# TopJohn/corda

Measured on AMD Instinct MI355X. Metric: signature verifications/sec (whole node, 1/2/4/8 GPU) + % integer-ALU peak, higher is better.
Workload: dtype u32

## Files before the change

### corda_amd/csrc/ed25519.hip

```cpp
#ifndef FE_QUAD
#define FE_QUAD 0
#endif
#ifndef FE_USE_ASM2
#define FE_USE_ASM2 1
#endif
#include <hip/hip_runtime.h>

#include <functional>
#include <stdint.h>
#include <stdlib.h>

#include "ed25519_ops.hpp"
#include "ed25519_ws.hpp"
#include "sha2_device.hpp"
#include "status.hpp"

namespace cordahip {

__global__ void __launch_bounds__(64) ed25519_btable_kernel(uint32_t* __restrict__ tab) {
  const int g = blockIdx.x * blockDim.x + threadIdx.x;
  if (g >= 2 * kBTableEntries) return;
  const int k = g % kBTableEntries;
  ge_p3 B, P;
  ge_base(B);
  if (g >= kBTableEntries)
    for (int t = 0; t < kBDigits * kBBits; t++) ge_dbl<true>(B, B);
  ge_cached bc;
  ge_to_cached(bc, B);
  ge_identity(P);
  for (int bit = kBBits - 1; bit >= 0; bit--) {
    ge_dbl<true>(P, P);
    if ((k >> bit) & 1) ge_add<true>(P, P, bc);
  }
  store_niels_entry(tab + g * kBEntryWords, P);
}

CDEV bool mp8_ge(const uint32_t a[8], const uint32_t b[8]) {
  uint32_t br = 0;
#pragma unroll
  for (int i = 0; i < 8; i++) br = (uint32_t)(((uint64_t)a[i] - b[i] - br) >> 63);
  return br == 0;
}
CDEV void mp8_add(uint32_t r[8], const uint32_t a[8], const uint32_t b[8]) {
  uint64_t c = 0;
#pragma unroll
  for (int i = 0; i < 8; i++) {
    c += (uint64_t)a[i] + b[i];
    r[i] = (uint32_t)c;
    c >>= 32;
  }
}
CDEV void mp8_neg(uint32_t a[8]) {
  uint64_t c = 1;
#pragma unroll
  for (int i = 0; i < 8; i++) {
    c += (uint64_t)(~a[i]);
    a[i] = (uint32_t)c;
    c >>= 32;
  }
}
CDEV void mp8_copy(uint32_t d[8], const uint32_t s[8]) {
#pragma unroll
  for (int i = 0; i < 8; i++) d[i] = s[i];
}
CDEV int mp8_absbits(const uint32_t a[8]) {
  uint32_t t[8];
  mp8_copy(t, a);
  if (a[7] >> 31) mp8_neg(t);
  return mp8_bitlen(t);
}

CDEV double mp8_f64(const uint32_t a[8]) {
  double d = (double)a[7];
#pragma unroll
  for (int i = 6; i >= 0; i--) d = fma(d, 4294967296.0, (double)a[i]);
  return d;
}
CDEV void mp8_submul(uint32_t a[8], const uint32_t b[8], uint32_t q) {
  uint64_t pc = 0;
  uint32_t br = 0;
#pragma unroll
  for (int i = 0; i < 8; i++) {
    const uint64_t p = (uint64_t)q * b[i] + pc;
    pc = p >> 32;
    const uint64_t d = (uint64_t)a[i] - (uint32_t)p - br;
    a[i] = (uint32_t)d;
    br = (uint32_t)(d >> 63);
  }
}
CDEV void mp8_shl_dyn(uint32_t o[8], const uint32_t b[8], int k) {
  const int ws = k >> 5, bs = k & 31;
#pragma unroll
  for (int i = 0; i < 8; i++) {
    const uint32_t lo = (i - ws >= 0) ? word_sel(b, i - ws) : 0u;
    const uint32_t lo2 = (i - ws - 1 >= 0) ? word_sel(b, i - ws - 1) : 0u;
    o[i] = bs ? ((lo << bs) | (lo2 >> (32 - bs))) : lo;
  }
}

CDEV void euclid_divstep(uint32_t rp[8], const uint32_t rc[8], uint32_t tp[8], const uint32_t tc[8]) {
  const double inv = 1.0 / mp8_f64(rc);
  while (mp8_ge(rp, rc)) {
    const double qd = mp8_f64(rp) * inv * (1.0 - 0x1p-40);
    if (qd < 4294967296.0) {
      uint32_t q = (uint32_t)qd;
      q = q ? q : 1u;
      mp8_submul(rp, rc, q);
      mp8_submul(tp, tc, q);
    } else {
      const int e = (int)((__double_as_longlong(qd) >> 52) & 0x7ff) - 1023;
      const int k = e - 31;
      const uint32_t q = (uint32_t)(qd * __longlong_as_double((long long)(1023 - k) << 52));
      uint32_t bs[8], ts[8];
      mp8_shl_dyn(bs, rc, k);
      mp8_shl_dyn(ts, tc, k);
      mp8_submul(rp, bs, q);
      mp8_submul(tp, ts, q);
    }
  }
}

CDEV double mp8_top(const uint32_t a[8], int s) {
  const int w = s >> 5, b = s & 31;
  const uint64_t lo = ((uint64_t)word_sel(a, w + 1) << 32) | word_sel(a, w);
  const uint64_t hi = word_sel(a, w + 2);
  return (double)((lo >> b) | (b ? hi << (64 - b) : 0ull));
}
CDEV void mp8_lincomb(uint32_t o[8], const uint32_t x[8], int a, const uint32_t y[8], int b) {
  const uint32_t ua = (uint32_t)(a < 0 ? -a : a), ub = (uint32_t)(b < 0 ? -b : b);
  uint64_t pc = 0, qc = 0;
  uint32_t br = 0;
#pragma unroll
  for (int i = 0; i < 8; i++) {
    const uint64_t p = (uint64_t)ua * x[i] + pc;
    pc = p >> 32;
    const uint64_t q = (uint64_t)ub * y[i] + qc;
    qc = q >> 32;
    const uint64_t d = (uint64_t)(uint32_t)p - (uint32_t)q - br;
    o[i] = (uint32_t)d;
    br = (uint32_t)(d >> 63);
  }
  if (b > 0 || (b == 0 && a < 0)) mp8_neg(o);
}

CDEV void half_scalars(uint32_t c0abs[8], bool& c0neg, uint32_t c1[8], const uint32_t h[8]) {
  const uint32_t kM[8] = {0xe7ae9f68u, 0xc09318d2u, 0x17bce6b2u, 0xa6f7cef5u, 0u, 0u, 0u, 0x80000000u};
  const uint32_t kS[8] = {0x754abea0u, 0x597d89b3u, 0xf9de6484u, 0xb504f333u, 0u, 0u, 0u, 0u};
  uint32_t rp[8], rc[8], tp[8], tc[8];
#pragma unroll
  for (int i = 0; i < 8; i++) {
    rp[i] = kM[i];
    rc[i] = h[i];
    tp[i] = 0;
    tc[i] = i == 0;
  }
  for (;;) {
    const int s = max(mp8_bitlen(rp) - 52, 0);
    double uh = mp8_top(rp, s), vh = mp8_top(rc, s);
    const double th = mp8_top(kS, s) + 1.0;
    double A = 1.0, B = 0.0, C = 0.0, D = 1.0;
    int n = 0;
    for (;;) {
      const double d1 = vh + C, d2 = vh + D;
      if (!(d1 > 0.0 && d2 > 0.0)) break;
      const double n1 = uh + A;
      double q = floor(n1 / d1);
      const double r1 = fma(-q, d1, n1);
      q = r1 < 0.0 ? q - 1.0 : (r1 >= d1 ? q + 1.0 : q);
      const double r2 = fma(-q, d2, uh + B);
      if (!(r2 >= 0.0 && r2 < d2)) break;
      const double nC = fma(-q, C, A), nD = fma(-q, D, B), nv = fma(-q, vh, uh);
      const double mc = fmax(fabs(nC), fabs(nD));
      if (nv - mc < th || mc >= 0x1p30) break;
      A = C;
      B = D;
      C = nC;
      D = nD;
      uh = vh;
      vh = nv;
      n++;
    }
    if (n == 0) break;
    const int a = (int)A, b = (int)B, c = (int)C, d = (int)D;
    uint32_t x[8], y[8];
    mp8_lincomb(x, rp, a, rc, b);
    mp8_lincomb(y, rp, c, rc, d);
    mp8_copy(rp, x);
    mp8_copy(rc, y);
    mp8_lincomb(x, tp, a, tc, b);
    mp8_lincomb(y, tp, c, tc, d);
    mp8_copy(tp, x);
    mp8_copy(tc, y);
  }
  while (mp8_ge(rc, kS)) {
    euclid_divstep(rp, rc, tp, tc);
#pragma unroll
    for (int i = 0; i < 8; i++) {
      const uint32_t a = rp[i], b = tp[i];
      rp[i] = rc[i];
      rc[i] = a;
      tp[i] = tc[i];
      tc[i] = b;
    }
  }
  uint32_t a0[8], a1[8];
  mp8_copy(a0, rc);
  mp8_copy(a1, tc);
  if (!(tc[0] & 1)) {
    uint32_t r3[8], t3[8];
    mp8_copy(r3, rp);
    mp8_copy(t3, tp);
    euclid_divstep(r3, rc, t3, tc);
    uint32_t p0[8], p1[8], m0[8], m1[8], nr3[8], nt3[8];
    mp8_add(p0, rc, r3);
    mp8_add(p1, tc, t3);
    mp8_copy(nr3, r3);
    mp8_neg(nr3);
    mp8_copy(nt3, t3);
    mp8_neg(nt3);
    mp8_add(m0, rc, nr3);
    mp8_add(m1, tc, nt3);
    int best = max(mp8_absbits(r3), mp8_absbits(t3));
    mp8_copy(a0, r3);
    mp8_copy(a1, t3);
    const int bp = max(mp8_absbits(p0), mp8_absbits(p1));
    if (bp < best) {
      best = bp;
      mp8_copy(a0, p0);
      mp8_copy(a1, p1);
    }
    const int bm = max(mp8_absbits(m0), mp8_absbits(m1));
    if (bm < best) {
      mp8_copy(a0, m0);
      mp8_copy(a1, m1);
    }
  }
  if (a1[7] >> 31) {
    mp8_neg(a0);
    mp8_neg(a1);
  }
  c0neg = (a0[7] >> 31) != 0;
  if (c0neg) mp8_neg(a0);
  mp8_copy(c0abs, a0);
  mp8_copy(c1, a1);
}

CDEV bool ge_strict_ok(const ge_p3& R, const uint32_t w[8]) {
  uint32_t all_ones = (w[7] & 0x7fffffffu) == 0x7fffffffu;
#pragma unroll
  for (int i = 1; i < 7; i++) all_ones &= (w[i] == 0xffffffffu);
  if (all_ones && w[0] >= 0xffffffedu) return false;
  return !((w[7] >> 31) && fe_iszero(R.X));
}

CDEV void store_point(uint32_t* __restrict__ o, const ge_p3& p) {
  uint4* o4 = reinterpret_cast<uint4*>(o);
  uint32_t w[32];
#pragma unroll
  for (int i = 0; i < 10; i++) {
    w[i] = p.X.v[i];
    w[10 + i] = p.Y.v[i];
    w[20 + i] = p.T.v[i];
  }
  w[30] = w[31] = 0;
#pragma unroll
  for (int q = 0; q < 8; q++) o4[q] = make_uint4(w[4 * q], w[4 * q + 1], w[4 * q + 2], w[4 * q + 3]);
}
CDEV void load_point(ge_p3& p, const uint32_t* __restrict__ o) {
  const uint4* o4 = reinterpret_cast<const uint4*>(o);
  uint32_t w[32];
#pragma unroll
  for (int q = 0; q < 8; q++) {
    const uint4 v = o4[q];
    w[4 * q] = v.x;
    w[4 * q + 1] = v.y;
    w[4 * q + 2] = v.z;
    w[4 * q + 3] = v.w;
  }
#pragma unroll
  for (int i = 0; i < 10; i++) {
    p.X.v[i] = w[i];
    p.Y.v[i] = w[10 + i];
    p.T.v[i] = w[20 + i];
  }
  fe_set(p.Z, 1);
}

static constexpr int kParkP = joint_index(2, 2), kParkQ = joint_index(2, -2);

CDEV uint32_t* joint_slot(uint32_t* rec, int idx) { return rec + kWhTab + idx * kWhEntryWords; }

CDEV void load_cached_niels(ge_niels& n, const uint32_t* __restrict__ p) {
  ge_cached c;
  load_cached(c, p);
  n.ypx = c.YpX;
  n.ymx = c.YmX;
  n.xy2d = c.T2d;
}

CDEV void joint_single_pass(uint32_t* __restrict__ rec, int pass) {
  ge_p3 B, D;
  load_point(B, joint_slot(rec, pass ? kParkQ : kParkP));
  ge_cached c;
  ge_to_cached(c, B);
  store_cached(joint_slot(rec, pass ? joint_index(0, 1) : joint_index(1, 0)), c);
  ge_dbl<true>(D, B);
  ge_to_cached(c, D);
  store_cached(joint_slot(rec, pass ? joint_index(0, 2) : joint_index(2, 0)), c);
}

CDEV void joint_sign_pass(uint32_t* __restrict__ rec, int s) {
  ge_p3 D, E;
  ge_niels nq, np;
  ge_cached c;
  load_point(D, joint_slot(rec, kParkP));
  load_cached_niels(nq, joint_slot(rec, joint_index(0, 1)));
  niels_cneg(nq, s < 0);
  ge_madd<true>(D, D, nq);
  ge_to_cached(c, D);
  store_cached(joint_slot(rec, joint_index(1, s)), c);
  ge_madd<true>(E, D, nq);
  ge_to_cached(c, E);
  store_cached(joint_slot(rec, joint_index(1, 2 * s)), c);
  load_cached_niels(np, joint_slot(rec, joint_index(1, 0)));
  ge_madd<true>(E, D, np);
  ge_to_cached(c, E);
  store_cached(joint_slot(rec, joint_index(2, s)), c);
  ge_dbl<true>(E, D);
  ge_to_cached(c, E);
  store_cached(joint_slot(rec, joint_index(2, 2 * s)), c);
}


#ifndef ED_PREP_WAVES
#define ED_PREP_WAVES 2
#endif
CDEV uint8_t prep_decode_phase(const uint8_t* __restrict__ keys, const uint8_t* __restrict__ sigs, uint64_t i,
                               uint32_t msg_len, const uint8_t* __restrict__ pre_status, uint32_t empty_is_error,
                               uint32_t* __restrict__ rec, uint32_t abyte[8], uint32_t Rw[8]) {
  uint8_t st = kStatusPending;
  load8(Rw, reinterpret_cast<const uint32_t*>(sigs + i * 64));
  {
    uint32_t wa[8];
    load8(wa, reinterpret_cast<const uint32_t*>(keys + i * 32));
    ge_p3 A, R;
    bool okA, okR;
    ge_frombytes_i2p_pair(A, okA, wa, R, okR, Rw);
    if (!okA) st = kStatusBadKey;
    else if (pre_status && pre_status[i] != kStatusOk) st = pre_status[i];
    else if (msg_len == 0 && empty_is_error) st = kStatusEmpty;
    fe_tobytes(abyte, A.Y);
    abyte[7] |= fe_isnegative(A.X) << 31;
    if (st == kStatusPending && !(okR && ge_strict_ok(R, Rw))) st = kStatusBadSig;
    if (st != kStatusPending) {
      ge_identity(A);
      ge_identity(R);
    }
    fe_neg(A.X, A.X);
    fe_neg(A.T, A.T);
    fe_neg(R.X, R.X);
    fe_neg(R.T, R.T);
    store_point(joint_slot(rec, kParkP), A);
    store_point(joint_slot(rec, kParkQ), R);
  }
  return st;
}

CDEV void prep_table_phase(uint32_t* __restrict__ rec) {
#pragma unroll 1
  for (int pass = 0; pass < 2; pass++) {
    joint_single_pass(rec, pass);
    PHASE_BARRIER();
  }
#pragma unroll 1
  for (int s = -1; s <= 1; s += 2) {
    joint_sign_pass(rec, s);
    PHASE_BARRIER();
  }
}

CDEV uint8_t prep_keys_phase(const uint8_t* __restrict__ keys, const uint8_t* __restrict__ sigs, uint64_t i,
                             uint32_t msg_len, const uint8_t* __restrict__ pre_status, uint32_t empty_is_error,
                             uint32_t* __restrict__ rec, uint32_t abyte[8], uint32_t Rw[8]) {
  const uint8_t st = prep_decode_phase(keys, sigs, i, msg_len, pre_status, empty_is_error, rec, abyte, Rw);
  PHASE_BARRIER();
  prep_table_phase(rec);
  return st;
}

CDEV void prep_msg_phase(const uint8_t* __restrict__ sigs, const uint8_t* __restrict__ msgs, uint32_t msg_len,
                         uint64_t i, uint8_t st, const uint32_t abyte[8], const uint32_t Rw[8],
                         uint32_t* __restrict__ rec) {
  uint32_t ka[8], kr[8], e[8];
  bool c0neg = false;
  if (st == kStatusPending) {
    uint32_t S[8], hd[16], h[8], se[8], zero[8];
    load8(S, reinterpret_cast<const uint32_t*>(sigs + i * 64 + 32));
    sha512_segments(hd, Rw, abyte, true, msgs + i * (uint64_t)msg_len, msg_len);
    sc_reduce512(h, hd);
    sc_effective_S(se, S, slide_drops_carry(S));
    half_scalars(ka, c0neg, kr, h);
#pragma unroll
    for (int q = 0; q < 8; q++) zero[q] = 0;
    sc_muladd(e, kr, se, zero);
  } else {
#pragma unroll
    for (int q = 0; q < 8; q++) ka[q] = kr[q] = e[q] = 0;
  }
  store8(rec + kWhKa, ka);
  store8(rec + kWhKr, kr);
  store8(rec + kWhE, e);
  reinterpret_cast<uint4*>(rec + kWhFlags)[0] = make_uint4(c0neg ? 1u : 0u, 0u, 0u, 0u);
}

__global__ void __launch_bounds__(256) __attribute__((amdgpu_waves_per_eu(ED_PREP_WAVES))) ed25519_prep_half_kernel(
    const uint8_t* __restrict__ keys, const uint8_t* __restrict__ sigs, const uint8_t* __restrict__ msgs,
    uint32_t msg_len, uint64_t base, uint64_t m, const uint8_t* __restrict__ pre_status,
    uint8_t* __restrict__ status, uint32_t* __restrict__ ws, uint32_t empty_is_error) {
  const uint64_t li = (uint64_t)blockIdx.x * blockDim.x + threadIdx.x;
  if (li >= m) return;
  const uint64_t i = base + li;
  uint32_t* rec = ws + li * kWhLaneWords;
  uint32_t abyte[8], Rw[8];
  const uint8_t st = prep_keys_phase(keys, sigs, i, msg_len, pre_status, empty_is_error, rec, abyte, Rw);
  prep_msg_phase(sigs, msgs, msg_len, i, st, abyte, Rw, rec);
  status[i] = st;
}

__global__ void __launch_bounds__(256) __attribute__((amdgpu_waves_per_eu(ED_PREP_WAVES))) ed25519_prep_keys_kernel(
    const uint8_t* __restrict__ keys, const uint8_t* __restrict__ sigs, uint32_t msg_len, uint64_t base, uint64_t m,
    const uint8_t* __restrict__ pre_status, uint8_t* __restrict__ status, uint32_t* __restrict__ ws,
    uint32_t empty_is_error) {
  const uint64_t li = (uint64_t)blockIdx.x * blockDim.x + threadIdx.x;
  if (li >= m) return;
  const uint64_t i = base + li;
  uint32_t* rec = ws + li * kWhLaneWords;
  uint32_t abyte[8], Rw[8];
  status[i] = prep_keys_phase(keys, sigs, i, msg_len, pre_status, empty_is_error, rec, abyte, Rw);
  store8(rec + kWhKa, abyte);
}

__global__ void __launch_bounds__(256) __attribute__((amdgpu_waves_per_eu(ED_PREP_WAVES))) ed25519_prep_msg_kernel(const uint8_t* __restrict__ sigs,
                                                               const uint8_t* __restrict__ msgs, uint32_t msg_len,
                                                               uint64_t base, uint64_t m,
                                                               const uint8_t* __restrict__ status,
                                                               uint32_t* __restrict__ ws) {
  const uint64_t li = (uint64_t)blockIdx.x * blockDim.x + threadIdx.x;
  if (li >= m) return;
  const uint64_t i = base + li;
  uint32_t* rec = ws + li * kWhLaneWords;
  uint32_t abyte[8], Rw[8];
  load8(abyte, rec + kWhKa);
  load8(Rw, reinterpret_cast<const uint32_t*>(sigs + i * 64));
  prep_msg_phase(sigs, msgs, msg_len, i, status[i], abyte, Rw, rec);
}

CDEV void fixed_base_mult(ge_p3& P, const uint32_t k[8], const uint32_t* __restrict__ btab) {
  ge_identity(P);
  for (int j = 31; j >= 0; j--) {
    if (j != 31) {
#pragma unroll
      for (int t = 0; t < 7; t++) ge_dbl<false>(P, P);
      ge_dbl<true>(P, P);
    }
    const int d = booth_digit<8>(k, j);
    ge_niels nb;
    load_niels(nb, btab, d < 0 ? -d : d);
    niels_cneg(nb, d < 0);
    ge_madd<true>(P, P, nb);
  }
}

__global__ void __launch_bounds__(256) ed25519_sign_kernel(const uint8_t* __restrict__ seeds,
                                                          const uint8_t* __restrict__ msgs, uint32_t msg_len,
                                                          uint64_t n, const uint32_t* __restrict__ btab,
                                                          uint8_t* __restrict__ pubs, uint8_t* __restrict__ sigs) {
  const uint64_t i = (uint64_t)blockIdx.x * blockDim.x + threadIdx.x;
  if (i >= n) return;
  uint32_t seed[8];
  {
    const uint4* s4 = reinterpret_cast<const uint4*>(seeds + i * 32);
    const uint4 a = s4[0], b = s4[1];
    seed[0] = a.x; seed[1] = a.y; seed[2] = a.z; seed[3] = a.w;
    seed[4] = b.x; seed[5] = b.y; seed[6] = b.z; seed[7] = b.w;
  }
  const uint8_t* msg = msgs + i * (uint64_t)msg_len;
  uint32_t hs[16], dummy[8];
#pragma unroll
  for (int q = 0; q < 8; q++) dummy[q] = 0;
  sha512_segments(hs, seed, dummy, false, msg, 0);
  uint32_t a[8], prefix[8];
#pragma unroll
  for (int q = 0; q < 8; q++) {
    a[q] = hs[q];
    prefix[q] = hs[8 + q];
  }
  a[0] &= ~7u;
  a[7] &= 0x3fffffffu;
  a[7] |= 0x40000000u;
  uint32_t a16[16], ar[8];
#pragma unroll
  for (int q = 0; q < 8; q++) {
    a16[q] = a[q];
    a16[8 + q] = 0;
  }
  sc_reduce512(ar, a16);
  ge_p3 A;
  fixed_base_mult(A, ar, btab);
  uint32_t pub[8];
  ge_tobytes(pub, A);
  uint32_t rh[16], r[8];
  sha512_segments(rh, prefix, dummy, false, msg, msg_len);
  sc_reduce512(r, rh);
  ge_p3 Rp;
  fixed_base_mult(Rp, r, btab);
  uint32_t R[8];
  ge_tobytes(R, Rp);
  uint32_t kh[16], k[8], S[8];
  sha512_segments(kh, R, pub, true, msg, msg_len);
  sc_reduce512(k, kh);
  sc_muladd(S, k, ar, r);
  uint4* p4 = reinterpret_cast<uint4*>(pubs + i * 32);
  p4[0] = make_uint4(pub[0], pub[1], pub[2], pub[3]);
  p4[1] = make_uint4(pub[4], pub[5], pub[6], pub[7]);
  uint4* s4 = reinterpret_cast<uint4*>(sigs + i * 64);
  s4[0] = make_uint4(R[0], R[1], R[2], R[3]);
  s4[1] = make_uint4(R[4], R[5], R[6], R[7]);
  s4[2] = make_uint4(S[0], S[1], S[2], S[3]);
  s4[3] = make_uint4(S[4], S[5], S[6], S[7]);
}

}

namespace cordahip {
hipError_t launch_ed25519_btable(uint32_t* tab, hipStream_t s) {
  hipLaunchKernelGGL(ed25519_btable_kernel, dim3((2 * kBTableEntries + 63) / 64), dim3(64), 0, s, tab);
  return hipGetLastError();
}
size_t ed25519_btable_bytes() { return 2 * (size_t)kBTableEntries * kBEntryWords * sizeof(uint32_t); }

size_t ed25519_ws_lane_bytes() { return kWhLaneWords * sizeof(uint32_t); }

hipError_t launch_ed25519_verify(const uint8_t* keys, const uint8_t* sigs, const uint8_t* msgs, uint32_t msg_len,
                                 uint64_t n, const uint32_t* btab, const uint8_t* pre_status, uint8_t* status,
                                 unsigned long long* verdict, uint32_t* ws, uint64_t ws_lanes, uint32_t flags,
                                 hipStream_t s, const std::function<hipError_t()>* before_msgs) {
  if (n == 0) return hipSuccess;
  if (!ws || ws_lanes < 64 || ws_lanes % 64) return hipErrorInvalidValue;
  bool msgs_ready = before_msgs == nullptr;
  for (uint64_t base = 0; base < n; base += ws_lanes) {
    const uint64_t m = n - base < ws_lanes ? n - base : ws_lanes;
    const uint32_t blocks = (uint32_t)((m + 255) / 256);
    hipError_t e = hipSuccess;
    if (msgs_ready) {
      hipLaunchKernelGGL(ed25519_prep_half_kernel, dim3(blocks), dim3(256), 0, s, keys, sigs, msgs, msg_len, base, m,
                         pre_status, status, ws, (flags & 1u) ? 0u : 1u);
      e = hipGetLastError();
    } else {
      hipLaunchKernelGGL(ed25519_prep_keys_kernel, dim3(blocks), dim3(256), 0, s, keys, sigs, msg_len, base, m,
                         pre_status, status, ws, (flags & 1u) ? 0u : 1u);
      e = hipGetLastError();
      e = e ? e : (*before_msgs)();
      msgs_ready = true;
      if (e == hipSuccess)
        hipLaunchKernelGGL(ed25519_prep_msg_kernel, dim3(blocks), dim3(256), 0, s, sigs, msgs, msg_len, base, m, status,
                           ws);
      e = e ? e : hipGetLastError();
    }
    if (e == hipSuccess) e = launch_ed25519_ladder(base, m, btab, ws, status, verdict, s);
    if (e != hipSuccess) return e;
  }
  return hipSuccess;
}

hipError_t launch_ed25519_sign(const uint8_t* seeds, const uint8_t* msgs, uint32_t msg_len, uint64_t n,
                               const uint32_t* btab, uint8_t* pubs, uint8_t* sigs, hipStream_t s) {
  if (n == 0) return hipSuccess;
  const uint64_t blocks = (n + 255) / 256;
  hipLaunchKernelGGL(ed25519_sign_kernel, dim3((uint32_t)blocks), dim3(256), 0, s, seeds, msgs, msg_len, n, btab,
                     pubs, sigs);
  return hipGetLastError();
}
}
```

### corda_amd/csrc/ed25519_ladder.hip

```cpp
#ifndef FE_USE_ASM2
#define FE_USE_ASM2 1
#endif
#include <hip/hip_runtime.h>
#include <stdint.h>

#include "ed25519_ws.hpp"
#include "status.hpp"

namespace cordahip {

__device__ __attribute__((aligned(64))) const uint32_t kIdentityCached[kWhEntryWords] = {1, 0, 0, 0, 0, 0, 0, 0, 0, 0,
                                                            1, 0, 0, 0, 0, 0, 0, 0, 0, 0,
                                                            1, 0, 0, 0, 0, 0, 0, 0, 0, 0,
                                                            0, 0, 0, 0, 0, 0, 0, 0, 0, 0};

#ifndef ED_LADDER_WAVES
#define ED_LADDER_WAVES 2
#endif
static_assert(512 / ED_LADDER_WAVES >= 168, "fe25519_asm.hpp's v160..v167 accumulators need >= 168 VGPRs per lane");

__global__ void __launch_bounds__(256) __attribute__((amdgpu_waves_per_eu(ED_LADDER_WAVES))) ed25519_ladder_half_kernel(
    uint64_t base, uint64_t m, const uint32_t* __restrict__ btab, const uint32_t* __restrict__ ws,
    uint8_t* __restrict__ status, unsigned long long* __restrict__ verdict) {
  const uint64_t li = (uint64_t)blockIdx.x * blockDim.x + threadIdx.x;
  const bool active = li < m;
  const uint64_t lc = active ? li : m - 1;
  const uint32_t* rec = ws + lc * kWhLaneWords;
  __shared__ uint32_t sk[24][256];
  const uint32_t* ska = &sk[0][threadIdx.x];
  const uint32_t* skr = &sk[8][threadIdx.x];
  const uint32_t* ske = &sk[16][threadIdx.x];
  int bits;
  {
    uint32_t ka[8], kr[8], e[8];
    load8(ka, rec + kWhKa);
    load8(kr, rec + kWhKr);
    load8(e, rec + kWhE);
#pragma unroll
    for (int q = 0; q < 8; q++) {
      sk[q][threadIdx.x] = ka[q];
      sk[8 + q][threadIdx.x] = kr[q];
      sk[16 + q][threadIdx.x] = e[q];
    }
    bits = max(mp8_bitlen(ka), mp8_bitlen(kr));
  }
  const bool c0neg = rec[kWhFlags] & 1u;
  const int W = max(wave_max((bits + 2) / 2), (kBDigits - 1) * (kBBits / 2) + 1);
  const uint32_t* btab2 = btab + kBTableEntries * kBEntryWords;
  ge_p3 P;
  ge_identity(P);
  for (int j = W - 1; j >= 0; j--) {
    const joint_sel sel = joint_select(joint_booth2(ska, 256, 8, j), joint_booth2(skr, 256, 8, j), c0neg);
    ge_cached c;
    load_cached(c, table_entry(rec, sel.idx));
    if (j != W - 1) {
      ge_dbl<false>(P, P);
      ge_dbl<true>(P, P);
    }
    cached_cneg(c, sel.neg);
    const bool bwin = j % (kBBits / 2) == 0 && j < kBDigits * (kBBits / 2);
    if (bwin) {
      const int d0 = booth_digit_col<kBBits>(ske, j / (kBBits / 2));
      const int d1 = booth_digit_col<kBBits>(ske, j / (kBBits / 2) + kBDigits);
      ge_niels nb0, nb1;
      load_niels(nb0, btab, d0 < 0 ? -d0 : d0);
      ge_add<true>(P, P, c);
      load_niels(nb1, btab2, d1 < 0 ? -d1 : d1);
      niels_cneg(nb0, d0 < 0);
      ge_madd<true>(P, P, nb0);
      niels_cneg(nb1, d1 < 0);
      ge_madd<false>(P, P, nb1);
    } else {
      ge_add<false>(P, P, c);
    }
  }
  fe d;
  fe_sub(d, P.Y, P.Z);
  const bool zero = fe_iszero(P.X) && fe_iszero(d);
  const uint64_t i = base + li;
  uint8_t st = kStatusBadSig;
  if (active) {
    st = status[i];
    if (st == kStatusPending) {
      st = zero ? kStatusOk : kStatusBadSig;
      status[i] = st;
    }
  }
  const unsigned long long ok = __ballot(active && st == kStatusOk);
  if ((threadIdx.x & 63) == 0 && active && verdict) verdict[i >> 6] = ok;
}

hipError_t launch_ed25519_ladder(uint64_t base, uint64_t m, const uint32_t* btab, const uint32_t* ws, uint8_t* status,
                                 unsigned long long* verdict, hipStream_t s) {
  const uint32_t blocks = (uint32_t)((m + 255) / 256);
  hipLaunchKernelGGL(ed25519_ladder_half_kernel, dim3(blocks), dim3(256), 0, s, base, m, btab, ws, status, verdict);
  return hipGetLastError();
}

}
```

### corda_amd/csrc/ed25519_ws.hpp

```cpp
#pragma once
#include "ed25519_joint.hpp"
#include "fe25519.hpp"
#include "ge25519.hpp"
#include "sc25519.hpp"

namespace cordahip {

static constexpr int kBBits = 16;
static constexpr int kBDigits = 8;
static constexpr int kBTableEntries = (1 << (kBBits - 1)) + 1;
static constexpr int kBEntryWords = 32;
static constexpr uint8_t kStatusPending = 0xff;

static constexpr int kWhEntryWords = 48;
static constexpr int kWhTab = 0;
static constexpr int kWhKa = kJointEntries * kWhEntryWords;
static constexpr int kWhKr = kWhKa + 8;
static constexpr int kWhE = kWhKa + 16;
static constexpr int kWhFlags = kWhKa + 24;
static constexpr int kWhLaneWords = kWhKa + 32;
static_assert(kWhLaneWords % 16 == 0, "records must start on 64-B sectors");

extern __device__ const uint32_t kIdentityCached[kWhEntryWords];

CDEV const uint32_t* table_entry(const uint32_t* rec, int idx) {
  return idx == kJointIdentity ? kIdentityCached : rec + kWhTab + idx * kWhEntryWords;
}

CDEV void load_niels(ge_niels& n, const uint32_t* __restrict__ tab, int idx) {
  const uint4* e = reinterpret_cast<const uint4*>(tab + idx * kBEntryWords);
  uint32_t w[32];
#pragma unroll
  for (int q = 0; q < 8; q++) {
    const uint4 v = e[q];
    w[4 * q] = v.x;
    w[4 * q + 1] = v.y;
    w[4 * q + 2] = v.z;
    w[4 * q + 3] = v.w;
  }
#pragma unroll
  for (int i = 0; i < 10; i++) {
    n.ypx.v[i] = w[i];
    n.ymx.v[i] = w[10 + i];
    n.xy2d.v[i] = w[20 + i];
  }
}

CDEV void niels_cneg(ge_niels& n, bool neg) {
  fe nt;
  fe_neg_loose(nt, n.xy2d);
#pragma unroll
  for (int i = 0; i < 10; i++) {
    const uint32_t a = n.ypx.v[i], b = n.ymx.v[i];
    n.ypx.v[i] = neg ? b : a;
    n.ymx.v[i] = neg ? a : b;
    n.xy2d.v[i] = neg ? nt.v[i] : n.xy2d.v[i];
  }
}
CDEV void cached_cneg(ge_cached& c, bool neg) {
  fe nt;
  fe_neg_loose(nt, c.T2d);
#pragma unroll
  for (int i = 0; i < 10; i++) {
    const uint32_t a = c.YpX.v[i], b = c.YmX.v[i];
    c.YpX.v[i] = neg ? b : a;
    c.YmX.v[i] = neg ? a : b;
    c.T2d.v[i] = neg ? nt.v[i] : c.T2d.v[i];
  }
}

CDEV void store_cached(uint32_t* __restrict__ o, const ge_cached& c) {
  uint4* o4 = reinterpret_cast<uint4*>(o);
  uint32_t w[40];
#pragma unroll
  for (int i = 0; i < 10; i++) {
    w[i] = c.YpX.v[i];
    w[10 + i] = c.YmX.v[i];
    w[20 + i] = c.Z.v[i];
    w[30 + i] = c.T2d.v[i];
  }
#pragma unroll
  for (int q = 0; q < 10; q++) o4[q] = make_uint4(w[4 * q], w[4 * q + 1], w[4 * q + 2], w[4 * q + 3]);
  o4[10] = o4[11] = make_uint4(0u, 0u, 0u, 0u);
}

CDEV void load_cached(ge_cached& c, const uint32_t* __restrict__ p) {
  const uint4* p4 = reinterpret_cast<const uint4*>(p);
  uint32_t w[40];
#pragma unroll
  for (int q = 0; q < 10; q++) {
    const uint4 v = p4[q];
    w[4 * q] = v.x;
    w[4 * q + 1] = v.y;
    w[4 * q + 2] = v.z;
    w[4 * q + 3] = v.w;
  }
#pragma unroll
  for (int i = 0; i < 10; i++) {
    c.YpX.v[i] = w[i];
    c.YmX.v[i] = w[10 + i];
    c.Z.v[i] = w[20 + i];
    c.T2d.v[i] = w[30 + i];
  }
}

CDEV void store8(uint32_t* __restrict__ o, const uint32_t v[8]) {
  uint4* o4 = reinterpret_cast<uint4*>(o);
  o4[0] = make_uint4(v[0], v[1], v[2], v[3]);
  o4[1] = make_uint4(v[4], v[5], v[6], v[7]);
}
CDEV void load8(uint32_t v[8], const uint32_t* __restrict__ p) {
  const uint4* p4 = reinterpret_cast<const uint4*>(p);
  const uint4 a = p4[0], b = p4[1];
  v[0] = a.x; v[1] = a.y; v[2] = a.z; v[3] = a.w; v[4] = b.x; v[5] = b.y; v[6] = b.z; v[7] = b.w;
}

CDEV int mp8_bitlen(const uint32_t a[8]) {
  int n = 0;
#pragma unroll
  for (int i = 0; i < 8; i++) n = a[i] ? 32 * i + 32 - __builtin_clz(a[i]) : n;
  return n;
}

template <int W>
CDEV int booth_digit_col(const uint32_t* col, int j) {
  const int lo = W * j - 1;
  uint32_t v;
  if (lo < 0) {
    v = (col[0] << 1) & ((1u << (W + 1)) - 1);
  } else {
    const int w = lo >> 5, sh = lo & 31;
    const uint64_t hi = w + 1 <= 7 ? col[(w + 1) * 256] : 0u;
    v = (uint32_t)(((hi << 32) | col[w * 256]) >> sh) & ((1u << (W + 1)) - 1);
  }
  return (int)((v + 1) >> 1) - (int)((v >> W) << W);
}

CDEV int wave_max(int v) {
#pragma unroll
  for (int o = 32; o > 0; o >>= 1) v = max(v, __shfl_xor(v, o));
  return v;
}

#define PHASE_BARRIER() __builtin_amdgcn_sched_barrier(0)

hipError_t launch_ed25519_ladder(uint64_t base, uint64_t m, const uint32_t* btab, const uint32_t* ws, uint8_t* status,
                                 unsigned long long* verdict, hipStream_t s);

}
```

Baseline: 113.7 million.

## Precompute per-window selector stream, park prep points in LDS, global identity entry

The prep kernel now Booth-recodes the two half-scalars and the base-point scalar once into a packed stream of 5-bit window selectors plus B-digit magnitudes and signs. The ladder kernel reads these from LDS instead of recomputing joint Booth digits at every window. Prep-phase parked points and niels values now live in a shared-memory column instead of the global workspace record, cutting global round trips. The identity cached entry is moved into the base table in global memory, and the niels padding words are loaded and kept live with an empty asm. Together this trades extra prep work and LDS use for less per-window integer work and fewer global accesses in the ladder, with some risk to occupancy.

Measured after the change: 116.3 million (median of 6 runs). 1.02x the previous value.

```diff
diff --git a/corda_amd/csrc/ed25519.hip b/corda_amd/csrc/ed25519.hip
--- a/corda_amd/csrc/ed25519.hip
+++ b/corda_amd/csrc/ed25519.hip
@@ -33,6 +33,14 @@
     if ((k >> bit) & 1) ge_add<true>(P, P, bc);
   }
   store_niels_entry(tab + g * kBEntryWords, P);
+  if (g == 0) {
+    ge_cached id;
+    fe_set(id.YpX, 1);
+    fe_set(id.YmX, 1);
+    fe_set(id.Z, 1);
+    fe_set(id.T2d, 0);
+    store_cached(tab + kBIdentityWord, id);
+  }
 }
 
 CDEV bool mp8_ge(const uint32_t a[8], const uint32_t b[8]) {
@@ -286,9 +294,24 @@
   fe_set(p.Z, 1);
 }
 
+#ifndef ED_PREP_LDS
+#define ED_PREP_LDS 1
+#endif
+#if !ED_PREP_LDS
 static constexpr int kParkP = joint_index(2, 2), kParkQ = joint_index(2, -2);
+#endif
+static constexpr int kPqT2d = 30, kPqQ = 40, kPqWords = 70;
 
 CDEV uint32_t* joint_slot(uint32_t* rec, int idx) { return rec + kWhTab + idx * kWhEntryWords; }
+
+CDEV void pq_store(uint32_t* col, int at, const fe& f) {
+#pragma unroll
+  for (int i = 0; i < 10; i++) col[(at + i) * 256] = f.v[i];
+}
+CDEV void pq_load(fe& f, const uint32_t* col, int at) {
+#pragma unroll
+  for (int i = 0; i < 10; i++) f.v[i] = col[(at + i) * 256];
+}
 
 CDEV void load_cached_niels(ge_niels& n, const uint32_t* __restrict__ p) {
   ge_cached c;
@@ -298,23 +321,73 @@
   n.xy2d = c.T2d;
 }
 
-CDEV void joint_single_pass(uint32_t* __restrict__ rec, int pass) {
+CDEV void park_point(uint32_t* __restrict__ rec, uint32_t* col, int which, const ge_p3& p) {
+#if ED_PREP_LDS
+  pq_store(col, which * kPqQ, p.X);
+  pq_store(col, which * kPqQ + 10, p.Y);
+  pq_store(col, which * kPqQ + 20, p.T);
+#else
+  store_point(joint_slot(rec, which ? kParkQ : kParkP), p);
+#endif
+}
+CDEV void load_parked(ge_p3& p, uint32_t* __restrict__ rec, const uint32_t* col, int which) {
+#if ED_PREP_LDS
+  pq_load(p.X, col, which * kPqQ);
+  pq_load(p.Y, col, which * kPqQ + 10);
+  pq_load(p.T, col, which * kPqQ + 20);
+  fe_set(p.Z, 1);
+#else
+  load_point(p, joint_slot(rec, which ? kParkQ : kParkP));
+#endif
+}
+CDEV void park_niels(uint32_t* col, int pass, const ge_cached& c) {
+#if ED_PREP_LDS
+  if (pass) {
+    pq_store(col, kPqQ, c.YpX);
+    pq_store(col, kPqQ + 10, c.YmX);
+    pq_store(col, kPqQ + 20, c.T2d);
+  } else {
+    pq_store(col, kPqT2d, c.T2d);
+  }
+#endif
+}
+CDEV void load_parked_niels(ge_niels& n, uint32_t* __restrict__ rec, const uint32_t* col, int which) {
+#if ED_PREP_LDS
+  if (which) {
+    pq_load(n.ypx, col, kPqQ);
+    pq_load(n.ymx, col, kPqQ + 10);
+    pq_load(n.xy2d, col, kPqQ + 20);
+  } else {
+    fe x, y;
+    pq_load(x, col, 0);
+    pq_load(y, col, 10);
+    fe_add(n.ypx, y, x);
+    fe_sub(n.ymx, y, x);
+    pq_load(n.xy2d, col, kPqT2d);
+  }
+#else
+  load_cached_niels(n, joint_slot(rec, which ? joint_index(0, 1) : joint_index(1, 0)));
+#endif
+}
+
+CDEV void joint_single_pass(uint32_t* __restrict__ rec, uint32_t* col, int pass) {
   ge_p3 B, D;
-  load_point(B, joint_slot(rec, pass ? kParkQ : kParkP));
+  load_parked(B, rec, col, pass);
   ge_cached c;
   ge_to_cached(c, B);
+  park_niels(col, pass, c);
   store_cached(joint_slot(rec, pass ? joint_index(0, 1) : joint_index(1, 0)), c);
   ge_dbl<true>(D, B);
   ge_to_cached(c, D);
   store_cached(joint_slot(rec, pass ? joint_index(0, 2) : joint_index(2, 0)), c);
 }
 
-CDEV void joint_sign_pass(uint32_t* __restrict__ rec, int s) {
+CDEV void joint_sign_pass(uint32_t* __restrict__ rec, uint32_t* col, int s) {
   ge_p3 D, E;
   ge_niels nq, np;
   ge_cached c;
-  load_point(D, joint_slot(rec, kParkP));
-  load_cached_niels(nq, joint_slot(rec, joint_index(0, 1)));
+  load_parked(D, rec, col, 0);
+  load_parked_niels(nq, rec, col, 1);
   niels_cneg(nq, s < 0);
   ge_madd<true>(D, D, nq);
   ge_to_cached(c, D);
@@ -322,7 +395,10 @@
   ge_madd<true>(E, D, nq);
   ge_to_cached(c, E);
   store_cached(joint_slot(rec, joint_index(1, 2 * s)), c);
-  load_cached_niels(np, joint_slot(rec, joint_index(1, 0)));
+#if ED_PREP_LDS
+  PHASE_BARRIER();
+#endif
+  load_parked_niels(np, rec, col, 0);
   ge_madd<true>(E, D, np);
   ge_to_cached(c, E);
   store_cached(joint_slot(rec, joint_index(2, s)), c);
@@ -337,7 +413,7 @@
 #endif
 CDEV uint8_t prep_decode_phase(const uint8_t* __restrict__ keys, const uint8_t* __restrict__ sigs, uint64_t i,
                                uint32_t msg_len, const uint8_t* __restrict__ pre_status, uint32_t empty_is_error,
-                               uint32_t* __restrict__ rec, uint32_t abyte[8], uint32_t Rw[8]) {
+                               uint32_t* __restrict__ rec, uint32_t* col, uint32_t abyte[8], uint32_t Rw[8]) {
   uint8_t st = kStatusPending;
   load8(Rw, reinterpret_cast<const uint32_t*>(sigs + i * 64));
   {
@@ -360,31 +436,31 @@
     fe_neg(A.T, A.T);
     fe_neg(R.X, R.X);
     fe_neg(R.T, R.T);
-    store_point(joint_slot(rec, kParkP), A);
-    store_point(joint_slot(rec, kParkQ), R);
+    park_point(rec, col, 0, A);
+    park_point(rec, col, 1, R);
   }
   return st;
 }
 
-CDEV void prep_table_phase(uint32_t* __restrict__ rec) {
+CDEV void prep_table_phase(uint32_t* __restrict__ rec, uint32_t* col) {
 #pragma unroll 1
   for (int pass = 0; pass < 2; pass++) {
-    joint_single_pass(rec, pass);
+    joint_single_pass(rec, col, pass);
     PHASE_BARRIER();
   }
 #pragma unroll 1
   for (int s = -1; s <= 1; s += 2) {
-    joint_sign_pass(rec, s);
+    joint_sign_pass(rec, col, s);
     PHASE_BARRIER();
   }
 }
 
 CDEV uint8_t prep_keys_phase(const uint8_t* __restrict__ keys, const uint8_t* __restrict__ sigs, uint64_t i,
                              uint32_t msg_len, const uint8_t* __restrict__ pre_status, uint32_t empty_is_error,
-                             uint32_t* __restrict__ rec, uint32_t abyte[8], uint32_t Rw[8]) {
-  const uint8_t st = prep_decode_phase(keys, sigs, i, msg_len, pre_status, empty_is_error, rec, abyte, Rw);
+                             uint32_t* __restrict__ rec, uint32_t* col, uint32_t abyte[8], uint32_t Rw[8]) {
+  const uint8_t st = prep_decode_phase(keys, sigs, i, msg_len, pre_status, empty_is_error, rec, col, abyte, Rw);
   PHASE_BARRIER();
-  prep_table_phase(rec);
+  prep_table_phase(rec, col);
   return st;
 }
 
@@ -407,11 +483,28 @@
 #pragma unroll
     for (int q = 0; q < 8; q++) ka[q] = kr[q] = e[q] = 0;
   }
+#if ED_SEL_STREAM
+  uint32_t sel[32];
+  sel_recode(sel, ka, kr, e, c0neg);
+  sel[kSelWords] = 0;
+  uint4* o4 = reinterpret_cast<uint4*>(rec + kWhSel);
+#pragma unroll
+  for (int q = 0; q < 8; q++) o4[q] = make_uint4(sel[4 * q], sel[4 * q + 1], sel[4 * q + 2], sel[4 * q + 3]);
+#else
   store8(rec + kWhKa, ka);
   store8(rec + kWhKr, kr);
   store8(rec + kWhE, e);
   reinterpret_cast<uint4*>(rec + kWhFlags)[0] = make_uint4(c0neg ? 1u : 0u, 0u, 0u, 0u);
-}
+#endif
+}
+
+#if ED_PREP_LDS
+#define PREP_PARK_COLUMN(col)                  \
+  __shared__ uint32_t pq_lds[kPqWords][256]; \
+  uint32_t* col = &pq_lds[0][threadIdx.x]
+#else
+#define PREP_PARK_COLUMN(col) uint32_t* col = nullptr
+#endif
 
 __global__ void __launch_bounds__(256) __attribute__((amdgpu_waves_per_eu(ED_PREP_WAVES))) ed25519_prep_half_kernel(
     const uint8_t* __restrict__ keys, const uint8_t* __restrict__ sigs, const uint8_t* __restrict__ msgs,
@@ -422,7 +515,8 @@
   const uint64_t i = base + li;
   uint32_t* rec = ws + li * kWhLaneWords;
   uint32_t abyte[8], Rw[8];
-  const uint8_t st = prep_keys_phase(keys, sigs, i, msg_len, pre_status, empty_is_error, rec, abyte, Rw);
+  PREP_PARK_COLUMN(col);
+  const uint8_t st = prep_keys_phase(keys, sigs, i, msg_len, pre_status, empty_is_error, rec, col, abyte, Rw);
   prep_msg_phase(sigs, msgs, msg_len, i, st, abyte, Rw, rec);
   status[i] = st;
 }
@@ -436,7 +530,8 @@
   const uint64_t i = base + li;
   uint32_t* rec = ws + li * kWhLaneWords;
   uint32_t abyte[8], Rw[8];
-  status[i] = prep_keys_phase(keys, sigs, i, msg_len, pre_status, empty_is_error, rec, abyte, Rw);
+  PREP_PARK_COLUMN(col);
+  status[i] = prep_keys_phase(keys, sigs, i, msg_len, pre_status, empty_is_error, rec, col, abyte, Rw);
   store8(rec + kWhKa, abyte);
 }
 
@@ -537,7 +632,7 @@
   hipLaunchKernelGGL(ed25519_btable_kernel, dim3((2 * kBTableEntries + 63) / 64), dim3(64), 0, s, tab);
   return hipGetLastError();
 }
-size_t ed25519_btable_bytes() { return 2 * (size_t)kBTableEntries * kBEntryWords * sizeof(uint32_t); }
+size_t ed25519_btable_bytes() { return ((size_t)kBIdentityWord + 64) * sizeof(uint32_t); }
 
 size_t ed25519_ws_lane_bytes() { return kWhLaneWords * sizeof(uint32_t); }
 
diff --git a/corda_amd/csrc/ed25519_ladder.hip b/corda_amd/csrc/ed25519_ladder.hip
--- a/corda_amd/csrc/ed25519_ladder.hip
+++ b/corda_amd/csrc/ed25519_ladder.hip
@@ -26,6 +26,70 @@
   const bool active = li < m;
   const uint64_t lc = active ? li : m - 1;
   const uint32_t* rec = ws + lc * kWhLaneWords;
+#if ED_IDENT_GLOBAL
+  const uint32_t* ident = btab + kBIdentityWord;
+#else
+  const uint32_t* ident = kIdentityCached;
+#endif
+  const uint32_t* btab2 = btab + kBTableEntries * kBEntryWords;
+  ge_p3 P;
+  ge_identity(P);
+#if ED_SEL_STREAM
+  __shared__ uint32_t sk[kSelWords][256];
+  {
+    const uint4* r4 = reinterpret_cast<const uint4*>(rec + kWhSel);
+#pragma unroll
+    for (int q = 0; q < (kSelWords + 3) / 4; q++) {
+      const uint4 v = r4[q];
+      const uint32_t w[4] = {v.x, v.y, v.z, v.w};
+#pragma unroll
+      for (int t = 0; t < 4; t++)
+        if (4 * q + t < kSelWords) sk[4 * q + t][threadIdx.x] = w[t];
+    }
+  }
+  const uint32_t* col = &sk[0][threadIdx.x];
+  const int W = min(max(wave_max((int)(col[kSelMeta * 256] >> 16)), (kBDigits - 1) * (kBBits / 2) + 1), kSelWindows);
+  uint32_t selw = col[((W - 1) / kSelPerWord) * 256];
+  for (int j = W - 1; j >= 0; j--) {
+    const int jn = max(j - 1, 0);
+    const uint32_t selw_next = col[(jn / kSelPerWord) * 256];
+    const uint32_t sel = selw >> (kSelBits * (j % kSelPerWord));
+    const uint32_t idx = sel & 15u;
+    const bool neg = sel & kSelNeg;
+    ge_cached c;
+    load_cached(c, idx == kSelIdentity ? ident : rec + kWhTab + idx * kWhEntryWords);
+    const bool bwin = j % (kBBits / 2) == 0 && j < kBDigits * (kBBits / 2);
+    uint32_t m0 = 0, m1 = 0, sg = 0;
+    const int t = j / (kBBits / 2);
+    if (bwin) {
+      m0 = col[(kSelMag + (t >> 1)) * 256];
+      m1 = col[(kSelMag + ((t + kBDigits) >> 1)) * 256];
+      sg = col[kSelMeta * 256];
+    }
+    if (j != W - 1) {
+      ge_dbl<false>(P, P);
+      ge_dbl<true>(P, P);
+    }
+    cached_cneg(c, neg);
+    if (bwin) {
+      const int sh = 16 * (t & 1);
+      ge_niels nb0, nb1;
+      uint32_t pad0[2], pad1[2];
+      load_niels(nb0, btab, (int)((m0 >> sh) & 0xffffu), pad0);
+      ge_add<true>(P, P, c);
+      load_niels(nb1, btab2, (int)((m1 >> sh) & 0xffffu), pad1);
+      niels_pad_use(pad0);
+      niels_cneg(nb0, (sg >> t) & 1u);
+      ge_madd<true>(P, P, nb0);
+      niels_pad_use(pad1);
+      niels_cneg(nb1, (sg >> (t + kBDigits)) & 1u);
+      ge_madd<false>(P, P, nb1);
+    } else {
+      ge_add<false>(P, P, c);
+    }
+    selw = selw_next;
+  }
+#else
   __shared__ uint32_t sk[24][256];
   const uint32_t* ska = &sk[0][threadIdx.x];
   const uint32_t* skr = &sk[8][threadIdx.x];
@@ -46,13 +110,10 @@
   }
   const bool c0neg = rec[kWhFlags] & 1u;
   const int W = max(wave_max((bits + 2) / 2), (kBDigits - 1) * (kBBits / 2) + 1);
-  const uint32_t* btab2 = btab + kBTableEntries * kBEntryWords;
-  ge_p3 P;
-  ge_identity(P);
   for (int j = W - 1; j >= 0; j--) {
     const joint_sel sel = joint_select(joint_booth2(ska, 256, 8, j), joint_booth2(skr, 256, 8, j), c0neg);
     ge_cached c;
-    load_cached(c, table_entry(rec, sel.idx));
+    load_cached(c, table_entry(rec, sel.idx, ident));
     if (j != W - 1) {
       ge_dbl<false>(P, P);
       ge_dbl<true>(P, P);
@@ -74,6 +135,7 @@
       ge_add<false>(P, P, c);
     }
   }
+#endif
   fe d;
   fe_sub(d, P.Y, P.Z);
   const bool zero = fe_iszero(P.X) && fe_iszero(d);
diff --git a/corda_amd/csrc/ed25519_sel.hpp b/corda_amd/csrc/ed25519_sel.hpp
--- /dev/null
+++ b/corda_amd/csrc/ed25519_sel.hpp
@@ -0,0 +1,90 @@
+#pragma once
+#include <stdint.h>
+
+#include "ed25519_joint.hpp"
+
+namespace cordahip {
+
+static constexpr int kSelPerWord = 6, kSelBits = 5;
+static constexpr int kSelWindows = 132;
+static constexpr uint32_t kSelIdentity = 15;
+static constexpr uint32_t kSelNeg = 16;
+static constexpr int kSelBDigits = 16;
+static constexpr int kSelMag = kSelWindows / kSelPerWord;
+static constexpr int kSelMeta = kSelMag + kSelBDigits / 2;
+static constexpr int kSelWords = kSelMeta + 1;
+static constexpr int kSelAlways = 80;
+static_assert(kSelWindows % kSelPerWord == 0 && kSelWindows >= 129 && kSelWords <= 32,
+              "the stream lives in the record's 32 scalar words");
+
+static constexpr uint32_t kBooth2Lut = 2u | 3u << 3 | 3u << 6 | 4u << 9 | 0u << 12 | 1u << 15 | 1u << 18 | 2u << 21;
+
+JOINT_HD uint32_t sel_byte(uint32_t va, uint32_t vr) {
+  const int ta = (int)((kBooth2Lut >> (3 * va)) & 7u), tr = (int)((kBooth2Lut >> (3 * vr)) & 7u);
+  const int s = 5 * ta + tr - 12;
+  const int m = s < 0 ? -s : s;
+  return ((uint32_t)(m - 1) & 15u) | (s < 0 ? kSelNeg : 0u);
+}
+static_assert(((uint32_t)kJointIdentity & 15u) == kSelIdentity && kJointEntries <= (int)kSelIdentity &&
+                  (kSelNeg | 15u) < (1u << kSelBits),
+              "selector encoding");
+
+JOINT_HD void sel_word(uint32_t out[kSelWords], int w, uint32_t a, uint32_t r, uint32_t pa, uint32_t pr) {
+#pragma unroll
+  for (int b = 0; b < 16; b++) {
+    const int j = 16 * w + b;
+    if (j >= kSelWindows) break;
+    const uint32_t va = b ? (a >> (2 * b - 1)) & 7u : ((a << 1) | pa) & 7u;
+    const uint32_t vr = b ? (r >> (2 * b - 1)) & 7u : ((r << 1) | pr) & 7u;
+    const int sh = kSelBits * (j % kSelPerWord);
+    out[j / kSelPerWord] ^= (sel_byte(va, vr) ^ (j >= kSelAlways ? kSelIdentity : 0u)) << sh;
+  }
+}
+
+JOINT_HD void sel_recode(uint32_t out[kSelWords], const uint32_t c0abs[8], const uint32_t c1[8], const uint32_t e[8],
+                         bool c0neg) {
+  const uint32_t flip = c0neg ? ~0u : 0u;
+#pragma unroll
+  for (int k = 0; k < kSelMag; k++) {
+    uint32_t v = 0;
+#pragma unroll
+    for (int t = 0; t < kSelPerWord; t++)
+      if (kSelPerWord * k + t >= kSelAlways) v |= kSelIdentity << (kSelBits * t);
+    out[k] = v;
+  }
+#pragma unroll
+  for (int w = 0; w < kSelAlways / 16; w++)
+    sel_word(out, w, c0abs[w] ^ flip, c1[w], w ? (c0abs[w - 1] ^ flip) >> 31 : flip >> 31, w ? c1[w - 1] >> 31 : 0u);
+  const uint32_t high = (c0abs[4] | c1[4]) >> 31 | c0abs[5] | c1[5] | c0abs[6] | c1[6] | c0abs[7] | c1[7];
+  if (high) {
+#pragma unroll
+    for (int w = kSelAlways / 16; w <= 8; w++)
+      sel_word(out, w, (w < 8 ? c0abs[w] : 0u) ^ flip, w < 8 ? c1[w] : 0u, (c0abs[w - 1] ^ flip) >> 31, c1[w - 1] >> 31);
+  }
+  uint32_t signs = 0;
+#pragma unroll
+  for (int w = 0; w < kSelBDigits / 2; w++) {
+    const uint32_t v0 = ((e[w] << 1) | (w ? e[w - 1] >> 31 : 0u)) & 0x1ffffu, v1 = e[w] >> 15;
+    const int d0 = (int)((v0 + 1) >> 1) - (int)((v0 >> 16) << 16), d1 = (int)((v1 + 1) >> 1) - (int)((v1 >> 16) << 16);
+    signs |= (d0 < 0 ? 1u : 0u) << (2 * w) | (d1 < 0 ? 1u : 0u) << (2 * w + 1);
+    out[kSelMag + w] = (uint32_t)(d0 < 0 ? -d0 : d0) | (uint32_t)(d1 < 0 ? -d1 : d1) << 16;
+  }
+  int bits = 0;
+#pragma unroll
+  for (int i = 0; i < 8; i++) {
+    const uint32_t m = c0abs[i] | c1[i];
+    bits = m ? 32 * i + 32 - __builtin_clz(m) : bits;
+  }
+  out[kSelMeta] = signs | (uint32_t)((bits + 2) / 2) << 16;
+}
+
+JOINT_HD uint32_t sel_window(const uint32_t s[kSelWords], int j) {
+  return (s[j / kSelPerWord] >> (kSelBits * (j % kSelPerWord))) & ((1u << kSelBits) - 1);
+}
+JOINT_HD int sel_count(const uint32_t s[kSelWords]) { return (int)((s[kSelMeta] >> 16) & 0xffu); }
+JOINT_HD int sel_bdigit(const uint32_t s[kSelWords], int t) {
+  const int mag = (int)((s[kSelMag + (t >> 1)] >> (16 * (t & 1))) & 0xffffu);
+  return (s[kSelMeta] >> t) & 1u ? -mag : mag;
+}
+
+}
diff --git a/corda_amd/csrc/ed25519_ws.hpp b/corda_amd/csrc/ed25519_ws.hpp
--- a/corda_amd/csrc/ed25519_ws.hpp
+++ b/corda_amd/csrc/ed25519_ws.hpp
@@ -1,5 +1,6 @@
 #pragma once
 #include "ed25519_joint.hpp"
+#include "ed25519_sel.hpp"
 #include "fe25519.hpp"
 #include "ge25519.hpp"
 #include "sc25519.hpp"
@@ -10,8 +11,16 @@
 static constexpr int kBDigits = 8;
 static constexpr int kBTableEntries = (1 << (kBBits - 1)) + 1;
 static constexpr int kBEntryWords = 32;
+static constexpr int kBIdentityWord = 2 * kBTableEntries * kBEntryWords;
+static_assert(kSelBDigits == 2 * kBDigits, "ed25519_sel.hpp recodes both halves of e");
 static constexpr uint8_t kStatusPending = 0xff;
 
+#ifndef ED_SEL_STREAM
+#define ED_SEL_STREAM 1
+#endif
+#ifndef ED_IDENT_GLOBAL
+#define ED_IDENT_GLOBAL 1
+#endif
 static constexpr int kWhEntryWords = 48;
 static constexpr int kWhTab = 0;
 static constexpr int kWhKa = kJointEntries * kWhEntryWords;
@@ -21,13 +30,15 @@
 static constexpr int kWhLaneWords = kWhKa + 32;
 static_assert(kWhLaneWords % 16 == 0, "records must start on 64-B sectors");
 
+static constexpr int kWhSel = kWhKa;
+
 extern __device__ const uint32_t kIdentityCached[kWhEntryWords];
 
-CDEV const uint32_t* table_entry(const uint32_t* rec, int idx) {
-  return idx == kJointIdentity ? kIdentityCached : rec + kWhTab + idx * kWhEntryWords;
+CDEV const uint32_t* table_entry(const uint32_t* rec, int idx, const uint32_t* ident) {
+  return idx == kJointIdentity ? ident : rec + kWhTab + idx * kWhEntryWords;
 }
 
-CDEV void load_niels(ge_niels& n, const uint32_t* __restrict__ tab, int idx) {
+CDEV void load_niels(ge_niels& n, const uint32_t* __restrict__ tab, int idx, uint32_t pad[2]) {
   const uint4* e = reinterpret_cast<const uint4*>(tab + idx * kBEntryWords);
   uint32_t w[32];
 #pragma unroll
@@ -44,6 +55,20 @@
     n.ymx.v[i] = w[10 + i];
     n.xy2d.v[i] = w[20 + i];
   }
+  pad[0] = w[30];
+  pad[1] = w[31];
+}
+CDEV void load_niels(ge_niels& n, const uint32_t* __restrict__ tab, int idx) {
+  uint32_t pad[2];
+  load_niels(n, tab, idx, pad);
+}
+#ifndef ED_NIELS_PAD_LIVE
+#define ED_NIELS_PAD_LIVE 1
+#endif
+CDEV void niels_pad_use(const uint32_t pad[2]) {
+#if ED_NIELS_PAD_LIVE
+  asm volatile("" ::"v"(pad[0]), "v"(pad[1]));
+#endif
 }
 
 CDEV void niels_cneg(ge_niels& n, bool neg) {
```
